# parca-dev/parca-agent

Measured on AMD Instinct MI355X. Metric: profiling_cpu_overhead_pct, lower is better.
Workload: dtype bf16; 1 GPU; model=llama3-8b, global_batch=1, seq_len=2048, parallelism=dp1, sampling_hz=19, node_cpus=256, cpu_samples=0, gpu_ring_events=94961, gpu_launch_stacks=4000, pc_samples=0, kernels_reported=5345

## Files before the change

### build_native.py

```python
#!/usr/bin/env python3

from __future__ import annotations

import argparse
import os
import shlex
import subprocess
import sys
import sysconfig
from pathlib import Path

REPO = Path(__file__).resolve().parent
CSRC = REPO / "csrc"
OUT = REPO / "parca_agent_amd" / "native"
ROCM = Path(os.environ.get("ROCM_PATH", "/opt/rocm"))
GFX_ARCH = os.environ.get("PYTORCH_ROCM_ARCH", "gfx950")

EXT_SUFFIX = sysconfig.get_config_var("EXT_SUFFIX") or ".so"


def _run(cmd: list[str]) -> None:
    print("+", " ".join(shlex.quote(c) for c in cmd), flush=True)
    subprocess.run(cmd, check=True, cwd=str(REPO))


def _pybind_includes() -> list[str]:
    import pybind11

    return [
        f"-I{pybind11.get_include()}",
        f"-I{sysconfig.get_path('include')}",
    ]


def _needs_build(target: Path, sources: list[Path]) -> bool:
    if not target.exists():
        return True
    t = target.stat().st_mtime
    return any(s.stat().st_mtime > t for s in sources)


def build_sampler(debug: bool = False, force: bool = False) -> Path:
    src = CSRC / "sampler" / "sampler.cc"
    out = OUT / f"_sampler{EXT_SUFFIX}"
    deps = [src, CSRC / "sampler" / "ehframe.cc"]
    if not force and not _needs_build(out, deps):
        return out
    opt = "-O1" if debug else "-O2"
    _run([
        "g++", opt, "-g", "-std=c++17", "-shared", "-fPIC",
        "-fvisibility=hidden", "-pthread",
        *_pybind_includes(),
        f"-I{CSRC}",
        str(src), "-o", str(out),
    ])
    return out


def build_rocprof_tool(debug: bool = False, force: bool = False) -> Path:
    src = CSRC / "rocprof" / "tool.cc"
    out = OUT / "libparca_rocprof.so"
    if not src.exists():
        return out
    if not force and not _needs_build(out, [src, CSRC / "rocprof" / "ring.h"]):
        return out
    opt = "-O1" if debug else "-O2"
    _run([
        str(ROCM / "bin" / "hipcc"), opt, "-g", "-std=c++17", "-shared",
        "-fPIC", "-pthread",
        f"-I{CSRC}",
        str(src),
        f"-L{ROCM}/lib", "-lrocprofiler-sdk",
        f"-Wl,-rpath,{ROCM}/lib",
        "-o", str(out),
    ])
    return out


def build_gpu(debug: bool = False, force: bool = False) -> Path:
    srcs = [CSRC / "gpu" / "gpu_module.cc", CSRC / "gpu" / "bucketize.hip",
            CSRC / "gpu" / "compact.hip"]
    srcs = [s for s in srcs if s.exists()]
    out = OUT / f"_gpu{EXT_SUFFIX}"
    if not srcs:
        return out
    deps = srcs + [CSRC / "gpu" / "bucketize.h", CSRC / "gpu" / "compact.h",
                   CSRC / "rocprof" / "ring.h"]
    if not force and not _needs_build(out, deps):
        return out
    opt = "-O1" if debug else "-O3"
    hipcc = str(ROCM / "bin" / "hipcc")
    _run([
        hipcc, opt, "-g", "-std=c++17", "-shared", "-fPIC",
        f"--offload-arch={GFX_ARCH}",
        "-fvisibility=hidden",
        *_pybind_includes(),
        f"-I{CSRC}",
        *[str(s) for s in srcs],
# ... 87 lines not shown
```

### csrc/sampler/sampler.cc

```cpp

#include <pybind11/pybind11.h>
#include <pybind11/stl.h>

#include <atomic>
#include <cerrno>
#include <cstdint>
#include <malloc.h>
#include <cstring>
#include <memory>
#include <mutex>
#include <stdexcept>
#include <string>
#include <thread>
#include <vector>

#include <fcntl.h>
#include <linux/perf_event.h>
#include <poll.h>
#include <sys/epoll.h>
#include <sys/ioctl.h>
#include <sys/mman.h>
#include <sys/syscall.h>
#include <unistd.h>

#include "sampler/ehframe.cc"

namespace py = pybind11;

namespace {

constexpr uint64_t kContextMin = static_cast<uint64_t>(-4095LL);
constexpr uint64_t kContextKernel = static_cast<uint64_t>(-128LL);
constexpr uint64_t kContextHV = static_cast<uint64_t>(-32LL);
constexpr uint64_t kContextGuestKernel = static_cast<uint64_t>(-2176LL);

long perf_event_open(struct perf_event_attr* attr, pid_t pid, int cpu,
                     int group_fd, unsigned long flags) {
  return syscall(SYS_perf_event_open, attr, pid, cpu, group_fd, flags);
}

struct SampleEvent {
  uint32_t pid = 0;
  uint32_t tid = 0;
  uint32_t cpu = 0;
  uint64_t time_ns = 0;
  std::vector<uint64_t> kernel_ips;
  std::vector<uint64_t> user_ips;
  std::vector<uint64_t> regs;
  std::shared_ptr<std::vector<uint8_t>> stack_arena;
  uint64_t stack_off = 0;
  uint64_t stack_len = 0;
  uint64_t stack_dyn_size = 0;
};

struct ProcEvent {
  int kind = 0;
  uint32_t pid = 0;
  uint32_t tid = 0;
  uint32_t ppid = 0;
  std::string comm;
  uint64_t addr = 0;
  uint64_t len = 0;
  uint64_t pgoff = 0;
  uint32_t prot = 0;
  std::string filename;
  uint64_t time_ns = 0;
};

struct Batch {
  std::vector<SampleEvent> samples;
  std::vector<ProcEvent> proc_events;
  std::shared_ptr<std::vector<uint8_t>> arena;
};

class RingBuffer {
 public:
  RingBuffer() = default;
  RingBuffer(const RingBuffer&) = delete;
  RingBuffer& operator=(const RingBuffer&) = delete;

  bool init(int fd, size_t data_pages) {
    size_t page = sysconf(_SC_PAGESIZE);
    size_ = (1 + data_pages) * page;
    void* m = mmap(nullptr, size_, PROT_READ | PROT_WRITE, MAP_SHARED, fd, 0);
    if (m == MAP_FAILED) return false;
    meta_ = static_cast<perf_event_mmap_page*>(m);
    data_ = static_cast<uint8_t*>(m) + page;
    data_size_ = data_pages * page;
    fd_ = fd;
    return true;
  }

  ~RingBuffer() {
    if (meta_) munmap(meta_, size_);
  }

  template <typename Fn>
  void drain(Fn&& cb) {
    uint64_t head = __atomic_load_n(&meta_->data_head, __ATOMIC_ACQUIRE);
    uint64_t tail = meta_->data_tail;
    while (tail < head) {
      auto* hdr = reinterpret_cast<perf_event_header*>(
          data_ + (tail & (data_size_ - 1)));
      size_t off = tail & (data_size_ - 1);
      const uint8_t* rec;
      if (off + hdr->size > data_size_) {
        scratch_.resize(hdr->size);
        size_t first = data_size_ - off;
        memcpy(scratch_.data(), data_ + off, first);
        memcpy(scratch_.data() + first, data_, hdr->size - first);
        rec = scratch_.data();
        hdr = reinterpret_cast<perf_event_header*>(scratch_.data());
      } else {
        rec = data_ + off;
      }
      cb(hdr->type, rec, hdr->size);
      tail += hdr->size;
    }
    __atomic_store_n(&meta_->data_tail, tail, __ATOMIC_RELEASE);
  }

  int fd() const { return fd_; }

 private:
  perf_event_mmap_page* meta_ = nullptr;
  uint8_t* data_ = nullptr;
  size_t data_size_ = 0;
  size_t size_ = 0;
  int fd_ = -1;
  std::vector<uint8_t> scratch_;
};

constexpr uint64_t kX86RegsMask = 0x3FFULL | (0xFFULL << 16);

class PerfSampler {
 public:
  PerfSampler(int freq, bool dwarf_stacks, uint32_t stack_dump_size,
              int ring_pages, bool track_mmaps, int target_pid)
      : freq_(freq),
        dwarf_(dwarf_stacks),
        stack_dump_(stack_dump_size),
        ring_pages_(ring_pages),
        track_mmaps_(track_mmaps),
        target_pid_(target_pid) {
    if (ring_pages_ <= 0 || (ring_pages_ & (ring_pages_ - 1)) != 0)
      throw std::invalid_argument("ring_pages must be a power of two");
  }

  ~PerfSampler() { stop(); }

  void start() {
    if (running_.exchange(true)) return;
    int ncpu = sysconf(_SC_NPROCESSORS_ONLN);
    epfd_ = epoll_create1(EPOLL_CLOEXEC);
    if (epfd_ < 0) throw std::runtime_error("epoll_create1 failed");

    rings_.clear();
    fds_.clear();
    rings_.reserve(ncpu);

    for (int cpu = 0; cpu < ncpu; ++cpu) {
      struct perf_event_attr attr;
      memset(&attr, 0, sizeof(attr));
      attr.size = sizeof(attr);
      attr.type = PERF_TYPE_SOFTWARE;
      attr.config = PERF_COUNT_SW_CPU_CLOCK;
      attr.freq = 1;
      attr.sample_freq = freq_;
      attr.sample_type = PERF_SAMPLE_TID | PERF_SAMPLE_TIME |
                         PERF_SAMPLE_CALLCHAIN | PERF_SAMPLE_CPU;
      if (dwarf_) {
        attr.sample_type |= PERF_SAMPLE_REGS_USER | PERF_SAMPLE_STACK_USER;
        attr.sample_regs_user = kX86RegsMask;
        attr.sample_stack_user = stack_dump_;
      }
      attr.disabled = 1;
      attr.inherit = 0;
      attr.exclude_hv = 1;
      attr.sample_max_stack = 127;
      attr.wakeup_events = 1;
      if (track_mmaps_) {
        attr.comm = 1;
        attr.task = 1;
        attr.mmap = 1;
        attr.mmap2 = 1;
        attr.mmap_data = 0;
      }

      int fd = perf_event_open(&attr, target_pid_, cpu, -1, PERF_FLAG_FD_CLOEXEC);
      if (fd < 0 && (errno == EACCES || errno == EPERM) && target_pid_ >= 0) {
        attr.exclude_kernel = 1;
        fd = perf_event_open(&attr, target_pid_, cpu, -1, PERF_FLAG_FD_CLOEXEC);
      }
      if (fd < 0) {
        if (errno == EACCES || errno == EPERM)
          throw std::runtime_error(
              "perf_event_open: permission denied (need root/CAP_PERFMON or "
              "kernel.perf_event_paranoid <= 1)");
        throw std::runtime_error(std::string("perf_event_open cpu ") +
                                 std::to_string(cpu) + ": " + strerror(errno));
      }
      auto ring = std::make_unique<RingBuffer>();
      if (!ring->init(fd, ring_pages_)) {
        close(fd);
        throw std::runtime_error("mmap of perf ring failed");
      }
      struct epoll_event ev;
      ev.events = EPOLLIN;
      ev.data.u32 = static_cast<uint32_t>(rings_.size());
      epoll_ctl(epfd_, EPOLL_CTL_ADD, fd, &ev);
      ioctl(fd, PERF_EVENT_IOC_ENABLE, 0);
      fds_.push_back(fd);
      rings_.push_back(std::move(ring));
    }

    drain_thread_ = std::thread([this] { drain_loop(); });
  }

  void stop() {
    if (!running_.exchange(false)) return;
    if (drain_thread_.joinable()) drain_thread_.join();
    for (int fd : fds_) {
      ioctl(fd, PERF_EVENT_IOC_DISABLE, 0);
      close(fd);
    }
    fds_.clear();
    rings_.clear();
    if (epfd_ >= 0) close(epfd_);
    epfd_ = -1;
  }

  Batch take() {
    Batch out;
    {
      std::lock_guard<std::mutex> lk(mu_);
      out.samples.swap(batch_.samples);
      out.proc_events.swap(batch_.proc_events);
      out.arena = std::move(batch_.arena);
      batch_.arena.reset();
    }
    return out;
  }

  uint64_t lost_count() const { return lost_.load(); }
  uint64_t sample_count() const { return nsamples_.load(); }
  uint64_t unknown_count() const { return unknown_.load(); }
  int n_cpus() const { return static_cast<int>(rings_.size()); }

 private:
  void drain_loop() {
    std::vector<struct epoll_event> events(rings_.size());
    while (running_.load(std::memory_order_relaxed)) {
      int n = epoll_wait(epfd_, events.data(), events.size(), 100);
      if (n < 0) {
        if (errno == EINTR) continue;
        break;
      }
      Batch local;
      for (auto& ring : rings_) {
        ring->drain([&](uint32_t type, const uint8_t* rec, size_t size) {
          decode(type, rec, size, local);
        });
      }
      if (!local.samples.empty() || !local.proc_events.empty()) {
        std::lock_guard<std::mutex> lk(mu_);
        auto& b = batch_;
        b.samples.insert(b.samples.end(),
                         std::make_move_iterator(local.samples.begin()),
                         std::make_move_iterator(local.samples.end()));
        b.proc_events.insert(b.proc_events.end(),
                             std::make_move_iterator(local.proc_events.begin()),
                             std::make_move_iterator(local.proc_events.end()));
        if (b.samples.size() > 1 << 20) {
          lost_ += b.samples.size();
          b.samples.clear();
        }
      }
    }
  }

  void decode(uint32_t type, const uint8_t* rec, size_t size, Batch& out) {
    const uint8_t* p = rec + sizeof(perf_event_header);
    const uint8_t* end = rec + size;
    auto rd64 = [&]() {
      uint64_t v;
      memcpy(&v, p, 8);
      p += 8;
      return v;
    };
    auto rd32 = [&]() {
      uint32_t v;
      memcpy(&v, p, 4);
      p += 4;
      return v;
    };

    switch (type) {
      case PERF_RECORD_SAMPLE: {
        SampleEvent ev;
        ev.pid = rd32();
        ev.tid = rd32();
        ev.time_ns = rd64();
        ev.cpu = rd32();
        rd32();
        uint64_t nr = rd64();
        if (nr > 512 || p + nr * 8 > end) {
          unknown_++;
          return;
        }
        bool in_kernel = true;
        for (uint64_t i = 0; i < nr; ++i) {
          uint64_t ip = rd64();
          if (ip >= kContextMin) {
            in_kernel = (ip == kContextKernel || ip == kContextHV ||
                         ip == kContextGuestKernel);
            continue;
          }
          (in_kernel ? ev.kernel_ips : ev.user_ips).push_back(ip);
        }
        if (dwarf_ && p < end) {
          uint64_t abi = rd64();
          if (abi != 0 ) {
            int nregs = __builtin_popcountll(kX86RegsMask);
            ev.regs.resize(nregs);
            for (int i = 0; i < nregs; ++i) ev.regs[i] = rd64();
          }
          if (p < end) {
            uint64_t stack_size = rd64();
            if (stack_size > 0 && p + stack_size <= end) {
              const uint8_t* stack_start = p;
              p += stack_size;
              uint64_t dyn = rd64();
              uint64_t keep = std::min<uint64_t>(dyn, stack_size);
              if (keep > 0) {
                if (!out.arena)
                  out.arena = std::make_shared<std::vector<uint8_t>>();
                ev.stack_arena = out.arena;
                ev.stack_off = out.arena->size();
                ev.stack_len = keep;
                out.arena->insert(out.arena->end(), stack_start,
                                  stack_start + keep);
              }
              ev.stack_dyn_size = dyn;
            }
          }
        }
        nsamples_++;
        out.samples.push_back(std::move(ev));
        break;
      }
      case PERF_RECORD_LOST: {
        rd64();
        lost_ += rd64();
        break;
      }
      case PERF_RECORD_COMM: {
        ProcEvent ev;
        ev.kind = 0;
        ev.pid = rd32();
        ev.tid = rd32();
        ev.comm.assign(reinterpret_cast<const char*>(p));
        out.proc_events.push_back(std::move(ev));
        break;
      }
      case PERF_RECORD_EXIT:
      case PERF_RECORD_FORK: {
        ProcEvent ev;
        ev.kind = (type == PERF_RECORD_EXIT) ? 2 : 3;
        ev.pid = rd32();
        ev.ppid = rd32();
        ev.tid = rd32();
        rd32();
        ev.time_ns = rd64();
        out.proc_events.push_back(std::move(ev));
        break;
      }
      case PERF_RECORD_MMAP2: {
        ProcEvent ev;
        ev.kind = 1;
        ev.pid = rd32();
        ev.tid = rd32();
        ev.addr = rd64();
        ev.len = rd64();
        ev.pgoff = rd64();
        rd64();
        rd64();
        rd64();
        ev.prot = rd32();
        rd32();
        ev.filename.assign(reinterpret_cast<const char*>(p));
        if (ev.prot & 0x4 ) out.proc_events.push_back(std::move(ev));
        break;
      }
      default:
        unknown_++;
    }
  }

  int freq_;
  bool dwarf_;
  uint32_t stack_dump_;
  int ring_pages_;
  bool track_mmaps_;
  int target_pid_;

  std::vector<std::unique_ptr<RingBuffer>> rings_;
  std::vector<int> fds_;
  int epfd_ = -1;
  std::atomic<bool> running_{false};
  std::thread drain_thread_;

  std::mutex mu_;
  Batch batch_;
  std::atomic<uint64_t> lost_{0}, nsamples_{0}, unknown_{0};
};


struct SwitchEvent {
  uint32_t pid = 0;
  uint32_t tid = 0;
  uint32_t cpu = 0;
  bool is_out = false;
  bool preempt = false;
  uint64_t time_ns = 0;
};

class OffCpuSampler {
 public:
  OffCpuSampler(uint64_t sample_period, int ring_pages)
      : period_(sample_period), ring_pages_(ring_pages) {}

  ~OffCpuSampler() { stop(); }

  void start() {
    if (running_.exchange(true)) return;
    int ncpu = sysconf(_SC_NPROCESSORS_ONLN);
    epfd_ = epoll_create1(EPOLL_CLOEXEC);
    for (int cpu = 0; cpu < ncpu; ++cpu) {
      struct perf_event_attr attr;
      memset(&attr, 0, sizeof(attr));
      attr.size = sizeof(attr);
      attr.type = PERF_TYPE_SOFTWARE;
      attr.config = PERF_COUNT_SW_CONTEXT_SWITCHES;
      attr.sample_period = period_;
      attr.sample_type = PERF_SAMPLE_TID | PERF_SAMPLE_TIME |
                         PERF_SAMPLE_CALLCHAIN | PERF_SAMPLE_CPU;
      attr.context_switch = 1;
      attr.sample_id_all = 1;
      attr.disabled = 1;
      attr.exclude_hv = 1;
      attr.sample_max_stack = 127;
      attr.wakeup_events = 64;
      int fd = perf_event_open(&attr, -1, cpu, -1, PERF_FLAG_FD_CLOEXEC);
      if (fd < 0) {
        if (cpu == 0)
          throw std::runtime_error(std::string("off-cpu event: ") +
                                   strerror(errno));
        continue;
      }
      auto ring = std::make_unique<RingBuffer>();
      if (!ring->init(fd, ring_pages_)) {
        close(fd);
        continue;
      }
      struct epoll_event ev;
      ev.events = EPOLLIN;
      ev.data.u32 = static_cast<uint32_t>(rings_.size());
      epoll_ctl(epfd_, EPOLL_CTL_ADD, fd, &ev);
      ioctl(fd, PERF_EVENT_IOC_ENABLE, 0);
      fds_.push_back(fd);
      rings_.push_back(std::move(ring));
    }
    drain_thread_ = std::thread([this] { drain_loop(); });
  }

  void stop() {
    if (!running_.exchange(false)) return;
    if (drain_thread_.joinable()) drain_thread_.join();
    for (int fd : fds_) {
      ioctl(fd, PERF_EVENT_IOC_DISABLE, 0);
      close(fd);
    }
    fds_.clear();
    rings_.clear();
    if (epfd_ >= 0) close(epfd_);
    epfd_ = -1;
  }

  std::pair<std::vector<SampleEvent>, std::vector<SwitchEvent>> take() {
    std::lock_guard<std::mutex> lk(mu_);
    auto out = std::make_pair(std::move(samples_), std::move(switches_));
    samples_.clear();
    switches_.clear();
    return out;
  }

  uint64_t lost() const { return lost_.load(); }

 private:
  void drain_loop() {
    std::vector<struct epoll_event> events(rings_.size() + 1);
    while (running_.load(std::memory_order_relaxed)) {
      int n = epoll_wait(epfd_, events.data(), events.size(), 100);
      if (n < 0 && errno != EINTR) break;
      std::vector<SampleEvent> ls;
      std::vector<SwitchEvent> lw;
      for (auto& ring : rings_) {
        ring->drain(
            [&](uint32_t type, const uint8_t* rec, size_t size) {
              decode(type, rec, size, ls, lw);
            });
      }
      if (!ls.empty() || !lw.empty()) {
        std::lock_guard<std::mutex> lk(mu_);
        samples_.insert(samples_.end(),
                        std::make_move_iterator(ls.begin()),
                        std::make_move_iterator(ls.end()));
        switches_.insert(switches_.end(), lw.begin(), lw.end());
        if (switches_.size() > 1 << 21) switches_.clear();
        if (samples_.size() > 1 << 18) samples_.clear();
      }
    }
  }

  void decode(uint32_t type, const uint8_t* rec, size_t size,
              std::vector<SampleEvent>& ls, std::vector<SwitchEvent>& lw) {
// ... 116 lines not shown
  void start() {
    if (running_.exchange(true)) return;
    int pmu_type = read_uprobe_pmu_type();
    if (pmu_type < 0)
      throw std::runtime_error("uprobe PMU unavailable "
                               "(/sys/bus/event_source/devices/uprobe)");
    int ret_bit = read_retprobe_bit();
    int ncpu = sysconf(_SC_NPROCESSORS_ONLN);
    epfd_ = epoll_create1(EPOLL_CLOEXEC);

    for (size_t si = 0; si < specs_.size(); ++si) {
      const Spec& spec = specs_[si];
      for (int cpu = 0; cpu < ncpu; ++cpu) {
        struct perf_event_attr attr;
        memset(&attr, 0, sizeof(attr));
        attr.size = sizeof(attr);
        attr.type = pmu_type;
        attr.config = spec.retprobe ? (1ULL << ret_bit) : 0;
        attr.config1 = reinterpret_cast<uint64_t>(spec.path.c_str());
        attr.config2 = spec.offset;
        attr.sample_period = 1;
        attr.sample_type = PERF_SAMPLE_TID | PERF_SAMPLE_TIME |
                           PERF_SAMPLE_CPU;
        attr.disabled = 1;
        attr.exclude_hv = 1;
        attr.wakeup_events = 1;
        int fd = perf_event_open(&attr, -1, cpu, -1, PERF_FLAG_FD_CLOEXEC);
        if (fd < 0) {
          if (cpu == 0)
            throw std::runtime_error(
                std::string("uprobe attach failed for ") + spec.path + ":" +
                std::to_string(spec.offset) + ": " + strerror(errno));
          continue;
        }
        auto ring = std::make_unique<RingBuffer>();
        if (!ring->init(fd, 8)) {
          close(fd);
          continue;
        }
        struct epoll_event ev;
        ev.events = EPOLLIN;
        ev.data.u32 = static_cast<uint32_t>(rings_.size());
        epoll_ctl(epfd_, EPOLL_CTL_ADD, fd, &ev);
        ioctl(fd, PERF_EVENT_IOC_ENABLE, 0);
        fds_.push_back(fd);
        ring_spec_.push_back(static_cast<uint32_t>(si));
        rings_.push_back(std::move(ring));
        uint32_t pair = spec.probe_id >> 1;
        pair_fds_[pair].push_back(fd);
        if (spec.max_rate)
          pair_rate_[pair] = std::max(pair_rate_[pair], spec.max_rate);
      }
    }
    drain_thread_ = std::thread([this] { drain_loop(); });
  }

  void stop() {
    if (!running_.exchange(false)) return;
    if (drain_thread_.joinable()) drain_thread_.join();
    for (int fd : fds_) {
      ioctl(fd, PERF_EVENT_IOC_DISABLE, 0);
      close(fd);
    }
    fds_.clear();
    rings_.clear();
    ring_spec_.clear();
    if (epfd_ >= 0) close(epfd_);
    epfd_ = -1;
  }

  std::vector<ProbeFire> take() {
    std::vector<ProbeFire> out;
    std::lock_guard<std::mutex> lk(mu_);
    out.swap(fires_);
    return out;
  }

  uint64_t lost() const { return lost_.load(); }
  int n_events() const { return static_cast<int>(fds_.size()); }
  uint64_t throttles() const { return throttles_.load(); }
  uint64_t throttled_fires() const { return throttled_fires_.load(); }

 private:
  struct Throttle {
    uint64_t win_start = 0;
    uint64_t count = 0;
    uint64_t disabled_until = 0;
    bool disabled = false;
  };

  static uint64_t mono_ns() {
    struct timespec ts;
    clock_gettime(CLOCK_MONOTONIC, &ts);
    return uint64_t(ts.tv_sec) * 1000000000ull + ts.tv_nsec;
  }

  void drain_loop() {
    std::vector<struct epoll_event> events(rings_.size() + 1);
    while (running_.load(std::memory_order_relaxed)) {
      int n = epoll_wait(epfd_, events.data(), events.size(), 100);
      if (n < 0 && errno != EINTR) break;
      uint64_t now = mono_ns();
      for (auto& [pair, th] : throttle_) {
        if (th.disabled && now >= th.disabled_until) {
          for (int fd : pair_fds_[pair]) ioctl(fd, PERF_EVENT_IOC_ENABLE, 0);
          th.disabled = false;
          th.win_start = now;
// ... 181 lines not shown
  py::class_<OffCpuSampler>(m, "OffCpuSampler")
      .def(py::init<uint64_t, int>(), py::arg("sample_period") = 100,
           py::arg("ring_pages") = 64)
      .def("start", &OffCpuSampler::start,
           py::call_guard<py::gil_scoped_release>())
      .def("stop", &OffCpuSampler::stop,
           py::call_guard<py::gil_scoped_release>())
      .def("take",
           [](OffCpuSampler& s) {
             std::pair<std::vector<SampleEvent>, std::vector<SwitchEvent>>
                 out;
             {
               py::gil_scoped_release rel;
               out = s.take();
             }
             return py::make_tuple(std::move(out.first),
                                   std::move(out.second));
           })
      .def_property_readonly("lost", &OffCpuSampler::lost);

  py::class_<ProbeFire>(m, "ProbeFire")
      .def_readonly("probe_id", &ProbeFire::probe_id)
      .def_readonly("pid", &ProbeFire::pid)
      .def_readonly("tid", &ProbeFire::tid)
      .def_readonly("cpu", &ProbeFire::cpu)
      .def_readonly("time_ns", &ProbeFire::time_ns)
      .def_readonly("is_return", &ProbeFire::is_return);

  py::class_<UprobeGroup>(m, "UprobeGroup")
      .def(py::init<const std::vector<
               std::tuple<std::string, uint64_t, bool, uint32_t,
                          uint64_t>>&>(),
           py::arg("specs"))
      .def("start", &UprobeGroup::start,
           py::call_guard<py::gil_scoped_release>())
      .def("stop", &UprobeGroup::stop,
           py::call_guard<py::gil_scoped_release>())
      .def("take",
           [](UprobeGroup& g) {
             std::vector<ProbeFire> out;
             {
               py::gil_scoped_release rel;
               out = g.take();
             }
             return out;
           })
      .def_property_readonly("lost", &UprobeGroup::lost)
      .def_property_readonly("n_events", &UprobeGroup::n_events)
      .def_property_readonly("throttles", &UprobeGroup::throttles)
      .def_property_readonly("throttled_fires",
                             &UprobeGroup::throttled_fires);

  py::class_<PerfSampler>(m, "PerfSampler")
      .def(py::init<int, bool, uint32_t, int, bool, int>(),
           py::arg("freq") = 19, py::arg("dwarf_stacks") = false,
           py::arg("stack_dump_size") = 16384, py::arg("ring_pages") = 64,
           py::arg("track_mmaps") = true, py::arg("target_pid") = -1)
      .def("start", &PerfSampler::start,
           py::call_guard<py::gil_scoped_release>())
      .def("stop", &PerfSampler::stop,
           py::call_guard<py::gil_scoped_release>())
      .def(
          "take",
          [](PerfSampler& s) {
            Batch b;
            {
              py::gil_scoped_release rel;
              b = s.take();
            }
            return py::make_tuple(std::move(b.samples),
                                  std::move(b.proc_events));
          })
      .def_property_readonly("lost", &PerfSampler::lost_count)
      .def_property_readonly("n_samples", &PerfSampler::sample_count)
      .def_property_readonly("unknown", &PerfSampler::unknown_count)
      .def_property_readonly("n_cpus", &PerfSampler::n_cpus);
}
```

### parca_agent_amd/cpu/service.py

```python

from __future__ import annotations

import logging
import threading
import time
from typing import Callable, List, Optional

from ..kallsyms import Kallsyms
from ..model import (
    Frame,
    FrameType,
    MappingFile,
    Trace,
    TraceEventMeta,
    TraceOrigin,
)
from ..procmaps import ExecutableCache, ProcessTable
from ..reporter.reporter import Reporter

log = logging.getLogger("parca_agent_amd.cpu")

KERNEL_MAPPING = MappingFile(path="[kernel.kallsyms]")
JIT_MAPPING = MappingFile(path="[jit]")

# ... 56 lines not shown
            unwinder.processes = self.processes
        self.python_unwinder = python_unwinder
        self.ruby_unwinder = ruby_unwinder
        self.jvm_unwinder = jvm_unwinder
        self.php_unwinder = php_unwinder
        self.python_stacks = 0
        self.ruby_stacks = 0
        self.jvm_stacks = 0
        self.php_stacks = 0
        self.perl_unwinder = None
        self.perl_stacks = 0
        from ..interp.perfmap import PerfMapResolver

        self.perf_maps = PerfMapResolver()
        from ..nativelabels import NativeLabelReader

        self.native_labels = NativeLabelReader()
        self._seen_executables: set = set()
        self._stop = threading.Event()
        self._thread: Optional[threading.Thread] = None
        from ..lru import LRU

        self._trace_cache: LRU = LRU(65536)
        self._frame_intern: LRU = LRU(262144)
        self.last_trace_by_pid: LRU = LRU(4096, ttl_seconds=600)
        self.samples_processed = 0
        self.samples_no_mapping = 0
        self.stacks_unwound_dwarf = 0
        self.trace_cache_hits = 0


    def start(self) -> None:
        self._sampler.start()
        self._stop.clear()
        self._thread = threading.Thread(
            target=self._run, name="cpu-sampler", daemon=True)
        self._thread.start()

    def stop(self) -> None:
        self._stop.set()
        if self._thread is not None:
            self._thread.join(timeout=10)
            self._thread = None
        self._sampler.stop()
        self._drain_once()

    @property
    def lost_samples(self) -> int:
        return self._sampler.lost

    @property
    def total_samples(self) -> int:
        return self._sampler.n_samples


    def _run(self) -> None:
        next_sweep = time.monotonic() + 60.0
        while not self._stop.wait(self.poll_interval):
            try:
                self._drain_once()
                now = time.monotonic()
                if now >= next_sweep:
                    next_sweep = now + 60.0
                    self.native_labels.sweep()
            except Exception:
                log.error("sample drain failed", exc_info=True)

    def _drain_once(self) -> None:
        samples, proc_events = self._sampler.take()
        for ev in proc_events:
            self.processes.handle_proc_event(ev)
            if ev.kind == 2 and ev.pid == ev.tid:
                self._drop_process_state(ev.pid)
        for s in samples:
            self._handle_sample(s)

    def _drop_process_state(self, pid: int) -> None:
        if self.unwinder is not None:
            self.unwinder.drop_process(pid)
        for interp in (self.python_unwinder, self.ruby_unwinder,
                       self.jvm_unwinder, self.php_unwinder,
                       self.perl_unwinder):
            if interp is not None and hasattr(interp, "drop_process"):
                interp.drop_process(pid)
        self.native_labels.forget(pid)


    def _handle_sample(self, s) -> None:
        if s.pid == 0:
            return

        user_ips = tuple(s.user_ips)
        if self.unwinder is not None and s.regs and s.stack and \
                len(user_ips) < 4:
            unwound = self.unwinder.unwind(s.pid, s.regs, s.stack)
            if len(unwound) > len(user_ips):
                user_ips = tuple(unwound)
                self.stacks_unwound_dwarf += 1

        py_frames: tuple = ()
        if self.python_unwinder is not None and \
                self.python_unwinder.available:
            sp = s.regs[7] if s.regs else 0
            py_frames = tuple(self.python_unwinder.stack_for(
                s.pid, s.tid, sp))
            if py_frames:
# ... 114 lines not shown
```

### parca_agent_amd/metrics.py

```python

from __future__ import annotations

from prometheus_client import CollectorRegistry
from prometheus_client.core import CounterMetricFamily, GaugeMetricFamily
from prometheus_client import ProcessCollector, PlatformCollector

from .version import __version__


class AgentCollector:
    def __init__(self, agent) -> None:
        self.agent = agent

    def collect(self):
        a = self.agent
        info = GaugeMetricFamily(
            "parca_agent_info", "Agent build info", labels=["version"])
        info.add_metric([__version__], 1)
        yield info

        rm = a.reporter.metrics
        c = CounterMetricFamily(
            "parca_agent_samples_ingested_total",
            "Samples ingested by the reporter", labels=["origin"])
        for origin, n in rm.samples_by_origin.items():
            c.add_metric([origin], n)
        yield c
        yield CounterMetricFamily(
            "parca_agent_samples_dropped_relabel_total",
            "Samples dropped by relabeling",
            value=rm.samples_dropped_relabel)
        yield CounterMetricFamily(
            "parca_agent_batches_written_total",
            "Flush batches written", value=rm.batches_written)
        yield CounterMetricFamily(
            "parca_agent_batch_errors_total",
            "Flush batch destination errors", value=rm.batch_errors)

        if a.cpu_service is not None:
            yield CounterMetricFamily(
                "parca_agent_cpu_samples_total",
                "perf samples decoded", value=a.cpu_service.total_samples)
            yield CounterMetricFamily(
                "parca_agent_cpu_samples_lost_total",
                "perf ring records lost", value=a.cpu_service.lost_samples)
            yield CounterMetricFamily(
                "parca_agent_cpu_samples_no_mapping_total",
                "sampled IPs without a mapping",
                value=a.cpu_service.samples_no_mapping)
            yield CounterMetricFamily(
                "parca_agent_dwarf_unwound_total",
                "stacks recovered by the .eh_frame unwinder",
                value=a.cpu_service.stacks_unwound_dwarf)
            uw = getattr(a.cpu_service, "unwinder", None)
            if uw is not None:
                yield CounterMetricFamily(
                    "parca_agent_dwarf_stacks_truncated_total",
                    "stacks truncated at the copied-stack-dump boundary",
                    value=uw._native.stacks_truncated)
                yield GaugeMetricFamily(
                    "parca_agent_dwarf_table_bytes",
                    "packed stack-delta table memory",
                    value=uw._native.total_bytes)
            interp = CounterMetricFamily(
                "parca_agent_interpreter_stacks_total",
                "samples with interpreter frames", labels=["runtime"])
            interp.add_metric(["python"], a.cpu_service.python_stacks)
            interp.add_metric(["ruby"], a.cpu_service.ruby_stacks)
            interp.add_metric(["jvm"], a.cpu_service.jvm_stacks)
            interp.add_metric(["php"], a.cpu_service.php_stacks)
            interp.add_metric(["perl"], a.cpu_service.perl_stacks)
            interp.add_metric(
                ["native_labels"],
                a.cpu_service.native_labels.samples_labeled)
            interp.add_metric(
                ["native_labels_read_errors"],
                a.cpu_service.native_labels.read_errors)
            yield interp

        if a.gpu_service is not None:
            if getattr(a.gpu_service, "hw_metrics", None) is not None:
                util = GaugeMetricFamily(
                    "parca_agent_gpu_utilization_percent",
                    "GPU busy percent (rocm-smi)", labels=["gpu"])
                vram = GaugeMetricFamily(
                    "parca_agent_gpu_vram_used_bytes",
                    "GPU VRAM used (rocm-smi)", labels=["gpu"])
                for s in a.gpu_service.hw_metrics.read():
                    if s.utilization_pct >= 0:
                        util.add_metric([str(s.gpu_index)],
                                        s.utilization_pct)
                    if s.vram_used_bytes >= 0:
                        vram.add_metric([str(s.gpu_index)],
                                        s.vram_used_bytes)
                yield util
# ... 61 lines not shown
```

Measured before the change: 0.08030 percent.

## Drain perf rings on watermark/timer with eventfd wake instead of per-event wakeups

Replaces wakeup_events=1 with a half-ring watermark, so the drain thread wakes on a timed sweep interval or when a specific ring fills, and then drains only the rings that signalled. The goal is to cut per-sample epoll wakeups and the full sweep over all 256 CPU rings on every wakeup. It also excludes idle samples in the kernel where supported, drops pid-0 samples early in the decoder, and hardens record parsing with bounds checks. In exchange, samples reach consumers with more latency, and an eventfd is added so stop() can still wake the thread promptly.

```diff
diff --git a/build_native.py b/build_native.py
--- a/build_native.py
+++ b/build_native.py
@@ -43,7 +43,8 @@
 def build_sampler(debug: bool = False, force: bool = False) -> Path:
     src = CSRC / "sampler" / "sampler.cc"
     out = OUT / f"_sampler{EXT_SUFFIX}"
-    deps = [src, CSRC / "sampler" / "ehframe.cc"]
+    deps = [src, CSRC / "sampler" / "ehframe.cc",
+            CSRC / "sampler" / "perf_ring.h"]
     if not force and not _needs_build(out, deps):
         return out
     opt = "-O1" if debug else "-O2"
diff --git a/csrc/sampler/perf_ring.h b/csrc/sampler/perf_ring.h
--- /dev/null
+++ b/csrc/sampler/perf_ring.h
@@ -0,0 +1,300 @@
+
+#pragma once
+
+#include <algorithm>
+#include <atomic>
+#include <cstdint>
+#include <cstring>
+#include <memory>
+#include <string>
+#include <vector>
+
+#include <linux/perf_event.h>
+#include <sys/mman.h>
+#include <unistd.h>
+
+namespace parca_perf {
+
+constexpr uint64_t kContextMin = static_cast<uint64_t>(-4095LL);
+constexpr uint64_t kContextKernel = static_cast<uint64_t>(-128LL);
+constexpr uint64_t kContextHV = static_cast<uint64_t>(-32LL);
+constexpr uint64_t kContextGuestKernel = static_cast<uint64_t>(-2176LL);
+
+constexpr uint64_t kX86RegsMask = 0x3FFULL | (0xFFULL << 16);
+
+constexpr uint64_t kMaxCallchain = 512;
+
+struct SampleEvent {
+  uint32_t pid = 0;
+  uint32_t tid = 0;
+  uint32_t cpu = 0;
+  uint64_t time_ns = 0;
+  std::vector<uint64_t> kernel_ips;
+  std::vector<uint64_t> user_ips;
+  std::vector<uint64_t> regs;
+  std::shared_ptr<std::vector<uint8_t>> stack_arena;
+  uint64_t stack_off = 0;
+  uint64_t stack_len = 0;
+  uint64_t stack_dyn_size = 0;
+};
+
+struct ProcEvent {
+  int kind = 0;
+  uint32_t pid = 0;
+  uint32_t tid = 0;
+  uint32_t ppid = 0;
+  std::string comm;
+  uint64_t addr = 0;
+  uint64_t len = 0;
+  uint64_t pgoff = 0;
+  uint32_t prot = 0;
+  std::string filename;
+  uint64_t time_ns = 0;
+};
+
+struct Batch {
+  std::vector<SampleEvent> samples;
+  std::vector<ProcEvent> proc_events;
+  std::shared_ptr<std::vector<uint8_t>> arena;
+};
+
+class RingBuffer {
+ public:
+  RingBuffer() = default;
+  RingBuffer(const RingBuffer&) = delete;
+  RingBuffer& operator=(const RingBuffer&) = delete;
+
+  bool init(int fd, size_t data_pages) {
+    size_t page = sysconf(_SC_PAGESIZE);
+    size_ = (1 + data_pages) * page;
+    void* m = mmap(nullptr, size_, PROT_READ | PROT_WRITE, MAP_SHARED, fd, 0);
+    if (m == MAP_FAILED) return false;
+    meta_ = static_cast<perf_event_mmap_page*>(m);
+    data_ = static_cast<uint8_t*>(m) + page;
+    data_size_ = data_pages * page;
+    fd_ = fd;
+    owns_map_ = true;
+    return true;
+  }
+
+  void init_from_memory(perf_event_mmap_page* meta, uint8_t* data,
+                        size_t data_size) {
+    meta_ = meta;
+    data_ = data;
+    data_size_ = data_size;
+    owns_map_ = false;
+  }
+
+  ~RingBuffer() {
+    if (meta_ && owns_map_) munmap(meta_, size_);
+  }
+
+  template <typename Fn>
+  void drain(Fn&& cb) {
+    uint64_t head = __atomic_load_n(&meta_->data_head, __ATOMIC_ACQUIRE);
+    uint64_t tail = meta_->data_tail;
+    if (tail == head) return;
+    while (tail < head) {
+      size_t off = tail & (data_size_ - 1);
+      perf_event_header hdr;
+      memcpy(&hdr, data_ + off, sizeof(hdr));
+      if (hdr.size < sizeof(hdr) || hdr.size > head - tail) {
+        tail = head;
+        break;
+      }
+      const uint8_t* rec;
+      if (off + hdr.size > data_size_) {
+        scratch_.resize(hdr.size);
+        size_t first = data_size_ - off;
+        memcpy(scratch_.data(), data_ + off, first);
+        memcpy(scratch_.data() + first, data_, hdr.size - first);
+        rec = scratch_.data();
+      } else {
+        rec = data_ + off;
+      }
+      cb(hdr.type, rec, hdr.size);
+      tail += hdr.size;
+    }
+    __atomic_store_n(&meta_->data_tail, tail, __ATOMIC_RELEASE);
+  }
+
+  int fd() const { return fd_; }
+
+ private:
+  perf_event_mmap_page* meta_ = nullptr;
+  uint8_t* data_ = nullptr;
+  size_t data_size_ = 0;
+  size_t size_ = 0;
+  int fd_ = -1;
+  bool owns_map_ = false;
+  std::vector<uint8_t> scratch_;
+};
+
+class RecordDecoder {
+ public:
+  explicit RecordDecoder(bool dwarf) : dwarf_(dwarf) {}
+
+  void decode(uint32_t type, const uint8_t* rec, size_t size, Batch& out) {
+    if (size < sizeof(perf_event_header)) {
+      unknown++;
+      return;
+    }
+    const uint8_t* p = rec + sizeof(perf_event_header);
+    const uint8_t* end = rec + size;
+    auto left = [&]() { return static_cast<uint64_t>(end - p); };
+    auto rd64 = [&]() {
+      uint64_t v;
+      memcpy(&v, p, 8);
+      p += 8;
+      return v;
+    };
+    auto rd32 = [&]() {
+      uint32_t v;
+      memcpy(&v, p, 4);
+      p += 4;
+      return v;
+    };
+    auto rdstr = [&](std::string& dst) {
+      dst.assign(reinterpret_cast<const char*>(p),
+                 strnlen(reinterpret_cast<const char*>(p), left()));
+    };
+
+    switch (type) {
+      case PERF_RECORD_SAMPLE: {
+        if (left() < 32) {
+          unknown++;
+          return;
+        }
+        uint32_t pid = rd32();
+        if (pid == 0) {
+          idle_dropped++;
+          return;
+        }
+        SampleEvent ev;
+        ev.pid = pid;
+        ev.tid = rd32();
+        ev.time_ns = rd64();
+        ev.cpu = rd32();
+        rd32();
+        uint64_t nr = rd64();
+        if (nr > kMaxCallchain || nr * 8 > left()) {
+          unknown++;
+          return;
+        }
+        bool in_kernel = true;
+        for (uint64_t i = 0; i < nr; ++i) {
+          uint64_t ip = rd64();
+          if (ip >= kContextMin) {
+            in_kernel = (ip == kContextKernel || ip == kContextHV ||
+                         ip == kContextGuestKernel);
+            continue;
+          }
+          (in_kernel ? ev.kernel_ips : ev.user_ips).push_back(ip);
+        }
+        if (dwarf_ && left() >= 8) {
+          uint64_t abi = rd64();
+          if (abi != 0 ) {
+            uint64_t nregs = __builtin_popcountll(kX86RegsMask);
+            if (nregs * 8 > left()) {
+              unknown++;
+              return;
+            }
+            ev.regs.resize(nregs);
+            for (uint64_t i = 0; i < nregs; ++i) ev.regs[i] = rd64();
+          }
+          if (left() >= 8) {
+            uint64_t stack_size = rd64();
+            if (stack_size > 0 && left() >= 8 && stack_size <= left() - 8) {
+              const uint8_t* stack_start = p;
+              p += stack_size;
+              uint64_t dyn = rd64();
+              uint64_t keep = std::min<uint64_t>(dyn, stack_size);
+              if (keep > 0) {
+                if (!out.arena)
+                  out.arena = std::make_shared<std::vector<uint8_t>>();
+                ev.stack_arena = out.arena;
+                ev.stack_off = out.arena->size();
+                ev.stack_len = keep;
+                out.arena->insert(out.arena->end(), stack_start,
+                                  stack_start + keep);
+              }
+              ev.stack_dyn_size = dyn;
+            }
+          }
+        }
+        nsamples++;
+        out.samples.push_back(std::move(ev));
+        break;
+      }
+      case PERF_RECORD_LOST: {
+        if (left() < 16) {
+          unknown++;
+          return;
+        }
+        rd64();
+        lost += rd64();
+        break;
+      }
+      case PERF_RECORD_COMM: {
+        if (left() < 8) {
+          unknown++;
+          return;
+        }
+        ProcEvent ev;
+        ev.kind = 0;
+        ev.pid = rd32();
+        ev.tid = rd32();
+        rdstr(ev.comm);
+        out.proc_events.push_back(std::move(ev));
+        break;
+      }
+      case PERF_RECORD_EXIT:
+      case PERF_RECORD_FORK: {
+        if (left() < 24) {
+          unknown++;
+          return;
+        }
+        ProcEvent ev;
+        ev.kind = (type == PERF_RECORD_EXIT) ? 2 : 3;
+        ev.pid = rd32();
+        ev.ppid = rd32();
+        ev.tid = rd32();
+        rd32();
+        ev.time_ns = rd64();
+        out.proc_events.push_back(std::move(ev));
+        break;
+      }
+      case PERF_RECORD_MMAP2: {
+        if (left() < 64) {
+          unknown++;
+          return;
+        }
+        ProcEvent ev;
+        ev.kind = 1;
+        ev.pid = rd32();
+        ev.tid = rd32();
+        ev.addr = rd64();
+        ev.len = rd64();
+        ev.pgoff = rd64();
+        rd64();
+        rd64();
+        rd64();
+        ev.prot = rd32();
+        rd32();
+        rdstr(ev.filename);
+        if (ev.prot & 0x4 )
+          out.proc_events.push_back(std::move(ev));
+        break;
+      }
+      default:
+        unknown++;
+    }
+  }
+
+  std::atomic<uint64_t> lost{0}, nsamples{0}, unknown{0}, idle_dropped{0};
+
+ private:
+  bool dwarf_;
+};
+
+}
diff --git a/csrc/sampler/sampler.cc b/csrc/sampler/sampler.cc
--- a/csrc/sampler/sampler.cc
+++ b/csrc/sampler/sampler.cc
@@ -4,6 +4,7 @@
 
 #include <atomic>
 #include <cerrno>
+#include <chrono>
 #include <cstdint>
 #include <malloc.h>
 #include <cstring>
@@ -17,147 +18,137 @@
 #include <fcntl.h>
 #include <linux/perf_event.h>
 #include <poll.h>
+#include <pthread.h>
 #include <sys/epoll.h>
+#include <sys/eventfd.h>
 #include <sys/ioctl.h>
 #include <sys/mman.h>
 #include <sys/syscall.h>
 #include <unistd.h>
 
 #include "sampler/ehframe.cc"
+#include "sampler/perf_ring.h"
 
 namespace py = pybind11;
 
 namespace {
 
-constexpr uint64_t kContextMin = static_cast<uint64_t>(-4095LL);
-constexpr uint64_t kContextKernel = static_cast<uint64_t>(-128LL);
-constexpr uint64_t kContextHV = static_cast<uint64_t>(-32LL);
-constexpr uint64_t kContextGuestKernel = static_cast<uint64_t>(-2176LL);
+using parca_perf::Batch;
+using parca_perf::ProcEvent;
+using parca_perf::RecordDecoder;
+using parca_perf::RingBuffer;
+using parca_perf::SampleEvent;
+using parca_perf::kContextGuestKernel;
+using parca_perf::kContextHV;
+using parca_perf::kContextKernel;
+using parca_perf::kContextMin;
+using parca_perf::kX86RegsMask;
 
 long perf_event_open(struct perf_event_attr* attr, pid_t pid, int cpu,
                      int group_fd, unsigned long flags) {
   return syscall(SYS_perf_event_open, attr, pid, cpu, group_fd, flags);
 }
 
-struct SampleEvent {
-  uint32_t pid = 0;
-  uint32_t tid = 0;
-  uint32_t cpu = 0;
-  uint64_t time_ns = 0;
-  std::vector<uint64_t> kernel_ips;
-  std::vector<uint64_t> user_ips;
-  std::vector<uint64_t> regs;
-  std::shared_ptr<std::vector<uint8_t>> stack_arena;
-  uint64_t stack_off = 0;
-  uint64_t stack_len = 0;
-  uint64_t stack_dyn_size = 0;
-};
-
-struct ProcEvent {
-  int kind = 0;
-  uint32_t pid = 0;
-  uint32_t tid = 0;
-  uint32_t ppid = 0;
-  std::string comm;
-  uint64_t addr = 0;
-  uint64_t len = 0;
-  uint64_t pgoff = 0;
-  uint32_t prot = 0;
-  std::string filename;
-  uint64_t time_ns = 0;
-};
-
-struct Batch {
-  std::vector<SampleEvent> samples;
-  std::vector<ProcEvent> proc_events;
-  std::shared_ptr<std::vector<uint8_t>> arena;
-};
-
-class RingBuffer {
- public:
-  RingBuffer() = default;
-  RingBuffer(const RingBuffer&) = delete;
-  RingBuffer& operator=(const RingBuffer&) = delete;
-
-  bool init(int fd, size_t data_pages) {
-    size_t page = sysconf(_SC_PAGESIZE);
-    size_ = (1 + data_pages) * page;
-    void* m = mmap(nullptr, size_, PROT_READ | PROT_WRITE, MAP_SHARED, fd, 0);
-    if (m == MAP_FAILED) return false;
-    meta_ = static_cast<perf_event_mmap_page*>(m);
-    data_ = static_cast<uint8_t*>(m) + page;
-    data_size_ = data_pages * page;
-    fd_ = fd;
-    return true;
-  }
-
-  ~RingBuffer() {
-    if (meta_) munmap(meta_, size_);
-  }
-
-  template <typename Fn>
-  void drain(Fn&& cb) {
-    uint64_t head = __atomic_load_n(&meta_->data_head, __ATOMIC_ACQUIRE);
-    uint64_t tail = meta_->data_tail;
-    while (tail < head) {
-      auto* hdr = reinterpret_cast<perf_event_header*>(
-          data_ + (tail & (data_size_ - 1)));
-      size_t off = tail & (data_size_ - 1);
-      const uint8_t* rec;
-      if (off + hdr->size > data_size_) {
-        scratch_.resize(hdr->size);
-        size_t first = data_size_ - off;
-        memcpy(scratch_.data(), data_ + off, first);
-        memcpy(scratch_.data() + first, data_, hdr->size - first);
-        rec = scratch_.data();
-        hdr = reinterpret_cast<perf_event_header*>(scratch_.data());
-      } else {
-        rec = data_ + off;
-      }
-      cb(hdr->type, rec, hdr->size);
-      tail += hdr->size;
-    }
-    __atomic_store_n(&meta_->data_tail, tail, __ATOMIC_RELEASE);
-  }
-
-  int fd() const { return fd_; }
-
- private:
-  perf_event_mmap_page* meta_ = nullptr;
-  uint8_t* data_ = nullptr;
-  size_t data_size_ = 0;
-  size_t size_ = 0;
-  int fd_ = -1;
-  std::vector<uint8_t> scratch_;
-};
-
-constexpr uint64_t kX86RegsMask = 0x3FFULL | (0xFFULL << 16);
-
 class PerfSampler {
  public:
   PerfSampler(int freq, bool dwarf_stacks, uint32_t stack_dump_size,
-              int ring_pages, bool track_mmaps, int target_pid)
+              int ring_pages, bool track_mmaps, int target_pid,
+              int drain_interval_ms)
       : freq_(freq),
         dwarf_(dwarf_stacks),
         stack_dump_(stack_dump_size),
         ring_pages_(ring_pages),
         track_mmaps_(track_mmaps),
-        target_pid_(target_pid) {
+        target_pid_(target_pid),
+        drain_interval_ms_(drain_interval_ms),
+        decoder_(dwarf_stacks) {
     if (ring_pages_ <= 0 || (ring_pages_ & (ring_pages_ - 1)) != 0)
       throw std::invalid_argument("ring_pages must be a power of two");
+    if (drain_interval_ms_ <= 0)
+      throw std::invalid_argument("drain_interval_ms must be positive");
   }
 
   ~PerfSampler() { stop(); }
 
   void start() {
     if (running_.exchange(true)) return;
+    try {
+      open_events();
+    } catch (...) {
+      close_all();
+      running_ = false;
+      throw;
+    }
+    drain_thread_ = std::thread([this] {
+      pthread_setname_np(pthread_self(), "perf-drain");
+      drain_loop();
+    });
+  }
+
+  void stop() {
+    if (!running_.exchange(false)) return;
+    if (wakefd_ >= 0) {
+      uint64_t one = 1;
+      ssize_t r = write(wakefd_, &one, sizeof(one));
+      (void)r;
+    }
+    if (drain_thread_.joinable()) drain_thread_.join();
+    for (int fd : fds_) ioctl(fd, PERF_EVENT_IOC_DISABLE, 0);
+    sweep_all();
+    close_all();
+  }
+
+  Batch take() {
+    Batch out;
+    {
+      std::lock_guard<std::mutex> lk(mu_);
+      out.samples.swap(batch_.samples);
+      out.proc_events.swap(batch_.proc_events);
+      out.arena = std::move(batch_.arena);
+      batch_.arena.reset();
+    }
+    return out;
+  }
+
+  uint64_t lost_count() const { return decoder_.lost.load(); }
+  uint64_t sample_count() const { return decoder_.nsamples.load(); }
+  uint64_t unknown_count() const { return decoder_.unknown.load(); }
+  uint64_t idle_dropped() const { return decoder_.idle_dropped.load(); }
+  uint64_t early_wakeups() const { return early_wakeups_.load(); }
+  uint64_t sweeps() const { return sweeps_.load(); }
+  int n_cpus() const { return static_cast<int>(rings_.size()); }
+
+ private:
+  static constexpr uint32_t kWakeToken = UINT32_MAX;
+
+  void close_all() {
+    for (int fd : fds_) close(fd);
+    fds_.clear();
+    rings_.clear();
+    if (wakefd_ >= 0) close(wakefd_);
+    wakefd_ = -1;
+    if (epfd_ >= 0) close(epfd_);
+    epfd_ = -1;
+  }
+
+  void open_events() {
     int ncpu = sysconf(_SC_NPROCESSORS_ONLN);
     epfd_ = epoll_create1(EPOLL_CLOEXEC);
     if (epfd_ < 0) throw std::runtime_error("epoll_create1 failed");
+    wakefd_ = eventfd(0, EFD_CLOEXEC | EFD_NONBLOCK);
+    if (wakefd_ < 0) throw std::runtime_error("eventfd failed");
+    {
+      struct epoll_event ev;
+      ev.events = EPOLLIN;
+      ev.data.u32 = kWakeToken;
+      epoll_ctl(epfd_, EPOLL_CTL_ADD, wakefd_, &ev);
+    }
 
     rings_.clear();
     fds_.clear();
     rings_.reserve(ncpu);
+    bool exclude_idle = target_pid_ < 0;
+    size_t page = sysconf(_SC_PAGESIZE);
 
     for (int cpu = 0; cpu < ncpu; ++cpu) {
       struct perf_event_attr attr;
@@ -178,7 +169,10 @@
       attr.inherit = 0;
       attr.exclude_hv = 1;
       attr.sample_max_stack = 127;
-      attr.wakeup_events = 1;
+      attr.watermark = 1;
+      attr.wakeup_watermark =
+          static_cast<uint32_t>(static_cast<size_t>(ring_pages_) * page / 2);
+      attr.exclude_idle = exclude_idle ? 1 : 0;
       if (track_mmaps_) {
         attr.comm = 1;
         attr.task = 1;
@@ -188,6 +182,11 @@
       }
 
       int fd = perf_event_open(&attr, target_pid_, cpu, -1, PERF_FLAG_FD_CLOEXEC);
+      if (fd < 0 && errno == EINVAL && attr.exclude_idle) {
+        exclude_idle = false;
+        attr.exclude_idle = 0;
+        fd = perf_event_open(&attr, target_pid_, cpu, -1, PERF_FLAG_FD_CLOEXEC);
+      }
       if (fd < 0 && (errno == EACCES || errno == EPERM) && target_pid_ >= 0) {
         attr.exclude_kernel = 1;
         fd = perf_event_open(&attr, target_pid_, cpu, -1, PERF_FLAG_FD_CLOEXEC);
@@ -213,187 +212,77 @@
       fds_.push_back(fd);
       rings_.push_back(std::move(ring));
     }
-
-    drain_thread_ = std::thread([this] { drain_loop(); });
-  }
-
-  void stop() {
-    if (!running_.exchange(false)) return;
-    if (drain_thread_.joinable()) drain_thread_.join();
-    for (int fd : fds_) {
-      ioctl(fd, PERF_EVENT_IOC_DISABLE, 0);
-      close(fd);
-    }
-    fds_.clear();
-    rings_.clear();
-    if (epfd_ >= 0) close(epfd_);
-    epfd_ = -1;
-  }
-
-  Batch take() {
-    Batch out;
-    {
-      std::lock_guard<std::mutex> lk(mu_);
-      out.samples.swap(batch_.samples);
-      out.proc_events.swap(batch_.proc_events);
-      out.arena = std::move(batch_.arena);
-      batch_.arena.reset();
-    }
-    return out;
-  }
-
-  uint64_t lost_count() const { return lost_.load(); }
-  uint64_t sample_count() const { return nsamples_.load(); }
-  uint64_t unknown_count() const { return unknown_.load(); }
-  int n_cpus() const { return static_cast<int>(rings_.size()); }
-
- private:
+  }
+
+  void drain_ring(RingBuffer& ring, Batch& local) {
+    ring.drain([&](uint32_t type, const uint8_t* rec, size_t size) {
+      decoder_.decode(type, rec, size, local);
+    });
+  }
+
+  void publish(Batch& local) {
+    if (local.samples.empty() && local.proc_events.empty()) return;
+    std::lock_guard<std::mutex> lk(mu_);
+    auto& b = batch_;
+    b.samples.insert(b.samples.end(),
+                     std::make_move_iterator(local.samples.begin()),
+                     std::make_move_iterator(local.samples.end()));
+    b.proc_events.insert(b.proc_events.end(),
+                         std::make_move_iterator(local.proc_events.begin()),
+                         std::make_move_iterator(local.proc_events.end()));
+    if (b.samples.size() > 1 << 20) {
+      decoder_.lost += b.samples.size();
+      b.samples.clear();
+    }
+  }
+
+  void sweep_all() {
+    Batch local;
+    for (auto& ring : rings_) drain_ring(*ring, local);
+    publish(local);
+  }
+
   void drain_loop() {
-    std::vector<struct epoll_event> events(rings_.size());
+    using clock = std::chrono::steady_clock;
+    const auto interval = std::chrono::milliseconds(drain_interval_ms_);
+    std::vector<struct epoll_event> events(rings_.size() + 1);
+    auto deadline = clock::now() + interval;
     while (running_.load(std::memory_order_relaxed)) {
-      int n = epoll_wait(epfd_, events.data(), events.size(), 100);
+      auto now = clock::now();
+      if (now >= deadline) {
+        sweep_all();
+        sweeps_++;
+        deadline += interval;
+        if (deadline <= now) deadline = now + interval;
+        continue;
+      }
+      auto left = std::chrono::duration_cast<std::chrono::milliseconds>(
+                      deadline - now).count() + 1;
+      int n = epoll_wait(epfd_, events.data(), events.size(),
+                         static_cast<int>(left));
       if (n < 0) {
         if (errno == EINTR) continue;
         break;
       }
+      if (n == 0) continue;
       Batch local;
-      for (auto& ring : rings_) {
-        ring->drain([&](uint32_t type, const uint8_t* rec, size_t size) {
-          decode(type, rec, size, local);
-        });
-      }
-      if (!local.samples.empty() || !local.proc_events.empty()) {
-        std::lock_guard<std::mutex> lk(mu_);
-        auto& b = batch_;
-        b.samples.insert(b.samples.end(),
-                         std::make_move_iterator(local.samples.begin()),
-                         std::make_move_iterator(local.samples.end()));
-        b.proc_events.insert(b.proc_events.end(),
-                             std::make_move_iterator(local.proc_events.begin()),
-                             std::make_move_iterator(local.proc_events.end()));
-        if (b.samples.size() > 1 << 20) {
-          lost_ += b.samples.size();
-          b.samples.clear();
+      bool ring_woke = false;
+      for (int i = 0; i < n; ++i) {
+        uint32_t token = events[i].data.u32;
+        if (token == kWakeToken) {
+          uint64_t v;
+          ssize_t r = read(wakefd_, &v, sizeof(v));
+          (void)r;
+          continue;
         }
-      }
-    }
-  }
-
-  void decode(uint32_t type, const uint8_t* rec, size_t size, Batch& out) {
-    const uint8_t* p = rec + sizeof(perf_event_header);
-    const uint8_t* end = rec + size;
-    auto rd64 = [&]() {
-      uint64_t v;
-      memcpy(&v, p, 8);
-      p += 8;
-      return v;
-    };
-    auto rd32 = [&]() {
-      uint32_t v;
-      memcpy(&v, p, 4);
-      p += 4;
-      return v;
-    };
-
-    switch (type) {
-      case PERF_RECORD_SAMPLE: {
-        SampleEvent ev;
-        ev.pid = rd32();
-        ev.tid = rd32();
-        ev.time_ns = rd64();
-        ev.cpu = rd32();
-        rd32();
-        uint64_t nr = rd64();
-        if (nr > 512 || p + nr * 8 > end) {
-          unknown_++;
-          return;
-        }
-        bool in_kernel = true;
-        for (uint64_t i = 0; i < nr; ++i) {
-          uint64_t ip = rd64();
-          if (ip >= kContextMin) {
-            in_kernel = (ip == kContextKernel || ip == kContextHV ||
-                         ip == kContextGuestKernel);
-            continue;
-          }
-          (in_kernel ? ev.kernel_ips : ev.user_ips).push_back(ip);
-        }
-        if (dwarf_ && p < end) {
-          uint64_t abi = rd64();
-          if (abi != 0 ) {
-            int nregs = __builtin_popcountll(kX86RegsMask);
-            ev.regs.resize(nregs);
-            for (int i = 0; i < nregs; ++i) ev.regs[i] = rd64();
-          }
-          if (p < end) {
-            uint64_t stack_size = rd64();
-            if (stack_size > 0 && p + stack_size <= end) {
-              const uint8_t* stack_start = p;
-              p += stack_size;
-              uint64_t dyn = rd64();
-              uint64_t keep = std::min<uint64_t>(dyn, stack_size);
-              if (keep > 0) {
-                if (!out.arena)
-                  out.arena = std::make_shared<std::vector<uint8_t>>();
-                ev.stack_arena = out.arena;
-                ev.stack_off = out.arena->size();
-                ev.stack_len = keep;
-                out.arena->insert(out.arena->end(), stack_start,
-                                  stack_start + keep);
-              }
-              ev.stack_dyn_size = dyn;
-            }
-          }
-        }
-        nsamples_++;
-        out.samples.push_back(std::move(ev));
-        break;
-      }
-      case PERF_RECORD_LOST: {
-        rd64();
-        lost_ += rd64();
-        break;
-      }
-      case PERF_RECORD_COMM: {
-        ProcEvent ev;
-        ev.kind = 0;
-        ev.pid = rd32();
-        ev.tid = rd32();
-        ev.comm.assign(reinterpret_cast<const char*>(p));
-        out.proc_events.push_back(std::move(ev));
-        break;
-      }
-      case PERF_RECORD_EXIT:
-      case PERF_RECORD_FORK: {
-        ProcEvent ev;
-        ev.kind = (type == PERF_RECORD_EXIT) ? 2 : 3;
-        ev.pid = rd32();
-        ev.ppid = rd32();
-        ev.tid = rd32();
-        rd32();
-        ev.time_ns = rd64();
-        out.proc_events.push_back(std::move(ev));
-        break;
-      }
-      case PERF_RECORD_MMAP2: {
-        ProcEvent ev;
-        ev.kind = 1;
-        ev.pid = rd32();
-        ev.tid = rd32();
-        ev.addr = rd64();
-        ev.len = rd64();
-        ev.pgoff = rd64();
-        rd64();
-        rd64();
-        rd64();
-        ev.prot = rd32();
-        rd32();
-        ev.filename.assign(reinterpret_cast<const char*>(p));
-        if (ev.prot & 0x4 ) out.proc_events.push_back(std::move(ev));
-        break;
-      }
-      default:
-        unknown_++;
+        if (token >= rings_.size()) continue;
+        drain_ring(*rings_[token], local);
+        ring_woke = true;
+        if (events[i].events & (EPOLLHUP | EPOLLERR))
+          epoll_ctl(epfd_, EPOLL_CTL_DEL, fds_[token], nullptr);
+      }
+      if (ring_woke) early_wakeups_++;
+      publish(local);
     }
   }
 
@@ -403,16 +292,19 @@
   int ring_pages_;
   bool track_mmaps_;
   int target_pid_;
+  int drain_interval_ms_;
 
   std::vector<std::unique_ptr<RingBuffer>> rings_;
   std::vector<int> fds_;
   int epfd_ = -1;
+  int wakefd_ = -1;
   std::atomic<bool> running_{false};
   std::thread drain_thread_;
 
   std::mutex mu_;
   Batch batch_;
-  std::atomic<uint64_t> lost_{0}, nsamples_{0}, unknown_{0};
+  RecordDecoder decoder_;
+  std::atomic<uint64_t> early_wakeups_{0}, sweeps_{0};
 };
 
 
@@ -471,7 +363,10 @@
       fds_.push_back(fd);
       rings_.push_back(std::move(ring));
     }
-    drain_thread_ = std::thread([this] { drain_loop(); });
+    drain_thread_ = std::thread([this] {
+      pthread_setname_np(pthread_self(), "offcpu-drain");
+      drain_loop();
+    });
   }
 
   void stop() {
@@ -694,7 +589,10 @@
           pair_rate_[pair] = std::max(pair_rate_[pair], spec.max_rate);
       }
     }
-    drain_thread_ = std::thread([this] { drain_loop(); });
+    drain_thread_ = std::thread([this] {
+      pthread_setname_np(pthread_self(), "uprobe-drain");
+      drain_loop();
+    });
   }
 
   void stop() {
@@ -982,10 +880,11 @@
                              &UprobeGroup::throttled_fires);
 
   py::class_<PerfSampler>(m, "PerfSampler")
-      .def(py::init<int, bool, uint32_t, int, bool, int>(),
+      .def(py::init<int, bool, uint32_t, int, bool, int, int>(),
            py::arg("freq") = 19, py::arg("dwarf_stacks") = false,
            py::arg("stack_dump_size") = 16384, py::arg("ring_pages") = 64,
-           py::arg("track_mmaps") = true, py::arg("target_pid") = -1)
+           py::arg("track_mmaps") = true, py::arg("target_pid") = -1,
+           py::arg("drain_interval_ms") = 100)
       .def("start", &PerfSampler::start,
            py::call_guard<py::gil_scoped_release>())
       .def("stop", &PerfSampler::stop,
@@ -1004,5 +903,8 @@
       .def_property_readonly("lost", &PerfSampler::lost_count)
       .def_property_readonly("n_samples", &PerfSampler::sample_count)
       .def_property_readonly("unknown", &PerfSampler::unknown_count)
+      .def_property_readonly("idle_dropped", &PerfSampler::idle_dropped)
+      .def_property_readonly("early_wakeups", &PerfSampler::early_wakeups)
+      .def_property_readonly("sweeps", &PerfSampler::sweeps)
       .def_property_readonly("n_cpus", &PerfSampler::n_cpus);
 }
diff --git a/parca_agent_amd/cpu/service.py b/parca_agent_amd/cpu/service.py
--- a/parca_agent_amd/cpu/service.py
+++ b/parca_agent_amd/cpu/service.py
@@ -132,6 +132,10 @@
     @property
     def total_samples(self) -> int:
         return self._sampler.n_samples
+
+    @property
+    def idle_dropped(self) -> int:
+        return self._sampler.idle_dropped
 
 
     def _run(self) -> None:
diff --git a/parca_agent_amd/metrics.py b/parca_agent_amd/metrics.py
--- a/parca_agent_amd/metrics.py
+++ b/parca_agent_amd/metrics.py
@@ -41,6 +41,10 @@
             yield CounterMetricFamily(
                 "parca_agent_cpu_samples_total",
                 "perf samples decoded", value=a.cpu_service.total_samples)
+            yield CounterMetricFamily(
+                "parca_agent_cpu_samples_idle_dropped_total",
+                "idle-task samples dropped in the native decoder",
+                value=a.cpu_service.idle_dropped)
             yield CounterMetricFamily(
                 "parca_agent_cpu_samples_lost_total",
                 "perf ring records lost", value=a.cpu_service.lost_samples)
```

Result: faster. 0.06380 percent (median of 5 runs) (-20.5%).
